# shionhonda/IaGo

Hardware: AMD Instinct MI355X
Metric: self-play games/sec (higher is better)
Workload: dtype f16 MFMA operands (float32 split in 2 / 3 pieces), f32 accumulate; u64 bitboards; f32 / f64 tree statistics

## Files before the change

iago_amd/csrc/search_kernel.hip:

```cpp
#include "mcts_dev.hpp"
#include "conv_trunk_body.hpp"
#include "conv_policy_body.hpp"
#include "sample_dev.hpp"
#include "search_request.hpp"
#include "../../include/iago_hip_serving.h"

#include <algorithm>
#include <cstdlib>
#include <mutex>
#include <string>
#include <vector>

namespace {
using namespace iago;
using namespace iago_mcts;

typedef unsigned long long u64;
#define RLX_AGENT __ATOMIC_RELAXED, __HIP_MEMORY_SCOPE_AGENT

constexpr uint32_t QCAP = IAGO_SEARCH_QUEUE_ENTRIES;
constexpr int CTL_FINISHED = 2, CTL_ABORT = 3;
__host__ __device__ constexpr int ctl_head(uint32_t q) { return 8 + 2 * (int)q; }
__host__ __device__ constexpr int ctl_tail(uint32_t q) { return 9 + 2 * (int)q; }
enum { ST_READY = 0, ST_WAIT_PRIOR, ST_PRIOR_READY, ST_ROLL, ST_ROLL_FRESH, ST_WAIT_VALUE, ST_HAVE_VALUE, ST_DONE, ST_TURN, ST_MOVE,
       ST_WAIT_DRAW, ST_DRAW,
       ST_IDLE };
constexpr int CTL_NO_CHILDREN = 4;
constexpr uint32_t MATCH_KEY = 0x4D415443u;
constexpr int CTL_BAD_DRAW = 13;
constexpr int CTL_PROGRESS = 5, CTL_PLAYING = 6;
constexpr int CTL_NET_WGS = 7;
constexpr int CTL_IDLE = 14;
constexpr int CTL_NEXT_GAME = 12;
namespace rq = iago_request;
using rq::KIND_POLICY;
using rq::KIND_VALUE;
using rq::NOBODY;
constexpr int GAMES_PER_WG = IAGO_SEARCH_GAMES_PER_WORKGROUP;

constexpr int SEARCH_IMG_V = iago_trunk::lds_alloc(2) + iago_trunk::head_lds(2);
constexpr int SEARCH_IMG_P = iago_policy::BS + 1024 + iago_policy::HEAD_FLOATS * 4;
constexpr int SEARCH_IMG_TOP = SEARCH_IMG_V > SEARCH_IMG_P ? SEARCH_IMG_V : SEARCH_IMG_P;

struct SearchParams {
    Tree T;
    const uint64_t *root_own, *root_opp;
    const uint8_t *active;
    float c_puct, lmbda;
    int32_t n_thr, n_sims, n_game_wgs, games_per_wg;
    int32_t *cur_node;
    uint64_t *cur_own, *cur_opp;
    int32_t *path;
    int32_t path_stride;
    int32_t *done;
    uint8_t *roll;
    int8_t *z;
    float *leaf_value;
    int8_t *z_log;
    int32_t *z_log_n;
    int32_t z_log_rows;
    u64 *q_slots;
    uint32_t *ctl;
    u64 *rep_v, *rep_p;
    int64_t *totals;
    int32_t *stats;
    uint64_t *wg_own, *wg_opp;
    long long clock_limit;
    int32_t max_turns;
    uint64_t *game_own, *game_opp;
    int32_t *n_turns;
    uint64_t *rec_own, *rec_opp;
    uint8_t *rec_valid;
    int8_t *rec_move;
    int32_t *rec_pi;
    int32_t games_total, stream;
    u64 *vtable;
    uint32_t vtable_mask;
    int64_t *trace;
    int32_t trace_rows;
    int32_t policy_xcds;
    int32_t pair_backlog;
    int32_t pace_margin, pace_backlog;
    int32_t ahead_idle;
    int32_t roll_defer;
    int32_t path_lds_cap;
    int32_t wave;
    float vloss;
    int64_t n_slots;
    int64_t *wave_timing;
    int32_t park_empties;
    uint8_t *parked;
    int32_t *park_stones;
    uint8_t *park_pass;
    int32_t explore_turns;
    int32_t cap_fast, cap_full_256;
    int32_t chain_skip;
    uint16_t *noise_counts;
    int32_t noise_eps, noise_lg;
    int32_t forced_k_256;
    int32_t negamax;
    float prior_off;
    double visit_off;
};

__device__ __forceinline__ u64 ld(const u64 *p) { return __hip_atomic_load(p, RLX_AGENT); }
__device__ __forceinline__ void st(u64 *p, u64 x) { __hip_atomic_store(p, x, RLX_AGENT); }

__device__ __forceinline__ u64 *ring_entry(const SearchParams &S, uint32_t q, uint32_t t)
{
    return S.q_slots + ((u64)q * QCAP + t % QCAP) * (u64)rq::SLOT_STRIDE;
}

__device__ __forceinline__ void send_request(const SearchParams &S, uint32_t kind, int64_t g, uint32_t reply_tag,
                                             uint64_t own, uint64_t opp)
{
    const uint32_t t = __hip_atomic_fetch_add(&S.ctl[ctl_tail(kind)], 1u, RLX_AGENT);
    u64 *e = S.q_slots + ((u64)kind * QCAP + t % QCAP) * (u64)rq::SLOT_STRIDE;
    st(e + rq::W_TAG, rq::entry_word(t, reply_tag));
    st(e + rq::W_OWN_LO, rq::entry_word(t, (uint32_t)own));
    st(e + rq::W_OWN_HI, rq::entry_word(t, (uint32_t)(own >> 32)));
    st(e + rq::W_OPP_LO, rq::entry_word(t, (uint32_t)opp));
    st(e + rq::W_OPP_HI, rq::entry_word(t, (uint32_t)(opp >> 32)));
    st(e + rq::W_WHO, rq::entry_word(t, rq::who_word(kind, (uint32_t)g)));
    atomicAdd((unsigned long long *)&S.totals[(uint32_t)g == NOBODY ? 11 : kind], 1ull);
}

__device__ __forceinline__ bool search_over(const SearchParams &S, const long long t0)
{
    bool out = false;
    if (threadIdx.x == 0)
        out = __hip_atomic_load(&S.ctl[CTL_FINISHED], RLX_AGENT) >= (uint32_t)S.n_game_wgs ||
              __hip_atomic_load(&S.ctl[CTL_ABORT], RLX_AGENT) != 0u || wall_clock64() - t0 > S.clock_limit;
    return __builtin_amdgcn_ballot_w64(out) != 0ull;
}

__device__ __forceinline__ int ring_backlog(const SearchParams &S, uint32_t q)
{
    int d = 0;
    if (threadIdx.x == 0)
        d = (int32_t)(__hip_atomic_load(&S.ctl[ctl_tail(q)], RLX_AGENT) - __hip_atomic_load(&S.ctl[ctl_head(q)], RLX_AGENT));
    return __builtin_amdgcn_readfirstlane(d);
}
__device__ __forceinline__ uint32_t ring_take(const SearchParams &S, uint32_t q)
{
    uint32_t t = 0;
    if (threadIdx.x == 0)
        t = __hip_atomic_fetch_add(&S.ctl[ctl_head(q)], 1u, RLX_AGENT);
    return __builtin_amdgcn_readfirstlane(t);
}
__device__ __forceinline__ int ring_fetch(const SearchParams &S, uint32_t q, uint32_t t, uint32_t max_spins, uint32_t *dst,
                                          const long long t0)
{
    const int tid = threadIdx.x;
    const u64 *e = ring_entry(S, q, t);
    u64 x = 0;
    int status = 0;
    for (uint32_t spins = 0;; spins++) {
        x = (tid < rq::WORDS) ? ld(e + tid) : 0ull;
        const bool ok = tid >= rq::WORDS || rq::entry_is(x, t);
        if (__builtin_amdgcn_ballot_w64(ok) == ~0ull)
            break;
        if (max_spins && spins + 1u >= max_spins) {
            status = 1;
            break;
        }
        if ((spins & 15u) == 15u && search_over(S, t0)) {
            status = 2;
            break;
        }
        __builtin_amdgcn_s_sleep(8);
    }
    if (status == 0 && tid < rq::WORDS)
        dst[tid] = (uint32_t)x;
    return status;
}

__device__ __forceinline__ void reply_value(const SearchParams &S, const uint32_t *r, uint32_t bits)
{
    if (rq::game(r) != NOBODY)
        st(&S.rep_v[(int64_t)rq::game(r)], rq::reply_word(rq::tag(r), bits));
}
__device__ __forceinline__ void reply_prior(const SearchParams &S, const uint32_t *r, int i, uint32_t bits)
{
    st(&S.rep_p[(int64_t)rq::game(r) * 64 + i], rq::reply_word(rq::tag(r), bits));
}

__device__ __forceinline__ uint32_t vtable_slot(const SearchParams &S, uint64_t own, uint64_t opp)
{
    uint64_t h = own * 0x9E3779B97F4A7C15ull ^ (opp + 0xD1B54A32D192ED03ull) * 0xBF58476D1CE4E5B9ull;
    h ^= h >> 29;
    h *= 0x94D049BB133111EBull;
    h ^= h >> 32;
    return (uint32_t)h & S.vtable_mask;
}

__device__ __forceinline__ bool vtable_get(const SearchParams &S, uint64_t own, uint64_t opp, uint32_t &bits, uint32_t &writer)
{
    const u64 *e = S.vtable + (u64)vtable_slot(S, own, opp) * 4u;
    const u64 s1 = ld(e), o = ld(e + 1), p = ld(e + 2), v = ld(e + 3);
    __builtin_amdgcn_fence(__ATOMIC_ACQUIRE, "wavefront");
    const u64 s2 = ld(e);
    bits = (uint32_t)v;
    writer = (uint32_t)(s1 >> 32);
    return s1 != 0ull && (s1 & 1ull) == 0ull && s1 == s2 && o == own && p == opp && (v >> 32) == (s1 & 0xFFFFFFFFull);
}

__device__ __forceinline__ u64 *vtable_put_begin(const SearchParams &S, uint64_t own, uint64_t opp, uint32_t bits, uint32_t writer,
                                                 u64 &publish)
{
    u64 *e = S.vtable + (u64)vtable_slot(S, own, opp) * 4u;
    const u64 s = __hip_atomic_fetch_or(e, 1ull, RLX_AGENT);
    if (s & 1ull)
        return nullptr;
    uint32_t seq = (uint32_t)s + 2u;
    seq = seq ? seq : 2u;
    st(e + 1, own);
    st(e + 2, opp);
    st(e + 3, ((u64)seq << 32) | bits);
    publish = ((u64)writer << 32) | seq;
    return e;
}
__device__ __forceinline__ void vtable_put_end(u64 *e, u64 publish)
{
    asm volatile("s_waitcnt vmcnt(0)" ::: "memory");
    st(e, publish);
}

template <int CTRL>
__device__ __forceinline__ void most_visited_step(int &n, int &a)
{
    const int on = (int)dpp_u32<CTRL>((uint32_t)n), oa = (int)dpp_u32<CTRL>((uint32_t)a);
    const bool take = on > n || (on == n && oa < a);
    n = take ? on : n;
    a = take ? oa : a;
}

__device__ __forceinline__ bool group8_all(bool x)
{
    return group8_add(x ? 0u : 1u) == 0u;
}

__device__ __forceinline__ int policy_draw(const u64 *rep, uint64_t lg, double u)
{
    double s = 0.0;
#pragma unroll 1
    for (int j = 0; j < 64; j++)
        s += ((lg >> j) & 1ull) ? (double)__uint_as_float(rq::reply_bits(ld(rep + j))) : 0.0;
    double last = 0.0;
#pragma unroll 1
    for (int j = 0; j < 64; j++)
        last += (((lg >> j) & 1ull) ? (double)__uint_as_float(rq::reply_bits(ld(rep + j))) : 0.0) / s;
    if (!(s > 0.0) || !(s <= 1.7976931348623157e308) || !(last > 0.0))
        return 64;
    double acc = 0.0;
    int n = 0;
#pragma unroll 1
    for (int j = 0; j < 64; j++) {
        acc += (((lg >> j) & 1ull) ? (double)__uint_as_float(rq::reply_bits(ld(rep + j))) : 0.0) / s;
        n += acc / last <= u ? 1 : 0;
    }
    return n;
}

__device__ __forceinline__ int path_entry(int path_at, const int32_t *gpath, int d)
{
    return path_at >= 0 ? ((const int32_t *)iago_trunk::trunk_lds)[path_at + d] : gpath[d];
}

template <bool WAVE>
__device__ __forceinline__ void backup_game(const SearchParams &S, int64_t g, uint32_t r, int leaf, bool fresh, float vg,
                                            int path_n, const int8_t zl, const int negamax, const int path_at,
                                            const int64_t gt)
{
    const int64_t base = gt * (int64_t)S.T.capacity;
    const float lmbda = S.lmbda;
    if (fresh && lmbda < 1.0f && r == 0u)
        S.T.nodes[base + leaf].v = vg;
    const int8_t zg = lmbda > 0.0f ? zl : (int8_t)0;
    const float lv = leaf_mix(lmbda, vg, zg);
    if (r == 0u) {
        S.leaf_value[g] = lv;
        if (S.z_log && lmbda > 0.0f)
            log_z(S.z_log, S.z_log_n, S.z_log_rows, gt, S.T.n_games, zg);
    }
    const int len = path_n < S.path_stride ? path_n : S.path_stride;
    const int32_t *const gpath = S.path + g * (int64_t)S.path_stride;
    const float lvd = backup_value(negamax, lv, path_n, (int)r);
    for (int d = (int)r; d < len; d += 8) {
        const int node = path_entry(path_at, gpath, d);
        visit(S.T, base + node, lvd);
        if constexpr (WAVE)
            S.T.nodes[base + node].reserved1 -= 1;
    }
}

__device__ __forceinline__ bool wg_handoff_or(bool x)
{
    __builtin_amdgcn_fence(__ATOMIC_RELEASE, "workgroup");
    const bool any = __syncthreads_or(x) != 0;
    __builtin_amdgcn_fence(__ATOMIC_ACQUIRE, "workgroup");
    return any;
}


struct Slot {
    int tid, gl;
    int wg;
    uint32_t r;
    Lane8 L;
    bool mine, exists;
    int64_t g, gt, base;
    int64_t n_slots;
    int W, s_in, tl;
    int path_at;
    int32_t *gpath;
    bool whole, need_v, need_z;
    int search_end;
};

struct Game {
    int state;
    uint32_t epoch;
    int n_done, turn, stones;
    bool pass_flg, g_over;
    uint64_t g_own, g_opp;
};

struct Cursor {
    int node, fc, k, nv, nvv;
    uint32_t vbits;
    uint64_t own, opp;
    int path_n, leaf;
    bool may_expand, leaf_fresh;
    float v_reply;
};

struct GameLds {
    uint64_t h_own[GAMES_PER_WG], h_opp[GAMES_PER_WG];
    int32_t h_stream[GAMES_PER_WG];
    int32_t h_game[GAMES_PER_WG];
    int32_t h_budget[GAMES_PER_WG];
    uint8_t h_fast[GAMES_PER_WG];
    uint32_t wg_count[7];
    int32_t ch_from[GAMES_PER_WG], ch_len[GAMES_PER_WG], ch_run[GAMES_PER_WG];
    int32_t roll_list[GAMES_PER_WG];
    uint32_t roll_wave[BLOCK / 64], roll_wave_old[BLOCK / 64];
    int32_t pace[4];
    uint32_t claimed;
    int32_t negamax;
    int8_t h_z[GAMES_PER_WG];
};
template <bool WAVE> struct GameShared : GameLds {};
template <> struct GameShared<true> : GameLds {
    int32_t wv_next[GAMES_PER_WG], wv_size[GAMES_PER_WG], wv_block[GAMES_PER_WG];
    long long wv_time[4];
};

template <bool WAVE>
__device__ __forceinline__ Slot make_slot(const SearchParams &S, const int wg)
{
    Slot I;
    I.wg = wg;
    I.tid = threadIdx.x;
    I.gl = I.tid >> 3;
    I.L = make_lane8(threadIdx.x);
    I.r = I.L.l8;
    I.mine = I.tid < 8 * S.games_per_wg;
    I.g = (int64_t)wg * S.games_per_wg + I.gl;
    I.W = WAVE ? S.wave : 1;
    I.n_slots = WAVE ? S.n_slots : S.T.n_games;
    I.exists = I.mine && I.g < I.n_slots;
    I.gt = WAVE ? I.g / I.W : I.g;
    I.s_in = WAVE ? (int)(I.g % I.W) : 0;
    I.tl = WAVE ? I.gl / I.W : 0;
    I.base = I.exists ? I.gt * (int64_t)S.T.capacity : 0;
    I.need_v = S.lmbda < 1.0f;
    I.need_z = S.lmbda > 0.0f;
    const bool path_lds = (size_t)S.games_per_wg * (size_t)S.path_stride * 4u <= (size_t)S.path_lds_cap;
    I.path_at = path_lds ? I.gl * S.path_stride : -1;
    I.gpath = S.path + (I.exists ? I.g : 0) * (int64_t)S.path_stride;
    I.whole = S.max_turns > 0;
    I.search_end = I.whole ? ST_MOVE : ST_DONE;
    return I;
}

__device__ __forceinline__ void start_game(Game &G, uint64_t own, uint64_t opp)
{
    G.g_own = own;
    G.g_opp = opp;
    G.turn = 0;
    G.stones = 4;
    G.pass_flg = false;
    G.g_over = false;
    G.n_done = 0;
}

template <bool WAVE>
__device__ __forceinline__ void cursor_to(Cursor &C, int node, uint32_t fc, uint32_t nv, uint32_t an, uint32_t vv, uint32_t vbits)
{
    C.node = node;
    C.fc = (int)fc;
    C.k = (int)((an >> 8) & 0xFFu);
    C.nv = (int)nv;
    if (WAVE)
        C.nvv = (int)vv;
    C.vbits = vbits;
}

__device__ __forceinline__ void finish_playout(const SearchParams &S, const Slot &I, const GameLds &sh, Game &G,
                                               const Cursor &C, bool fresh, float v)
{
    backup_game<false>(S, I.g, I.r, C.leaf, fresh, v, C.path_n, sh.h_z[I.gl], sh.negamax, I.path_at, I.g);
    G.n_done++;
    if (S.trace && I.r == 0u)
        atomicAdd((unsigned long long *)&S.totals[9], 1ull);
    if (I.r == 0u)
        S.done[I.g] = G.turn * S.n_sims + G.n_done;
    G.state = G.n_done >= sh.h_budget[I.gl] ? I.search_end : ST_READY;
}

__device__ __forceinline__ void take_replies(const SearchParams &S, const iago_row::HwParams &R, const Slot &I,
                                             const GameLds &sh, Game &G, Cursor &C)
{
    if (G.state == ST_WAIT_PRIOR || G.state == ST_WAIT_DRAW) {
        bool ok = true;
#pragma unroll
        for (int i = 0; i < 8; i++)
            ok = ok && rq::reply_tag(ld(&S.rep_p[I.g * 64 + (int)I.r * 8 + i])) == G.epoch;
        if (group8_all(ok)) {
            if (G.state == ST_WAIT_DRAW) {
                const uint64_t lg = group8_legal(to_lane(G.g_own, I.L), to_lane(G.g_opp, I.L), I.L);
                const double u = sample_uniform(R.key0, R.key1 ^ MATCH_KEY, R.id_base + (uint32_t)sh.h_game[I.gl],
                                                (uint32_t)G.turn, 0u);
                C.leaf = policy_draw(S.rep_p + I.g * 64, lg, u);
                if (C.leaf == 64) {
                    if (I.r == 0u)
                        __hip_atomic_store(&S.ctl[CTL_BAD_DRAW], 1u, RLX_AGENT);
                    C.leaf = (int)__builtin_ctzll(lg);
                }
            }
            G.state = G.state == ST_WAIT_PRIOR ? ST_PRIOR_READY : ST_DRAW;
        }
    } else if (G.state == ST_WAIT_VALUE) {
        const u64 x = ld(&S.rep_v[I.g]);
        if (rq::reply_tag(x) == G.epoch) {
            C.v_reply = __uint_as_float(rq::reply_bits(x));
            G.state = ST_HAVE_VALUE;
        }
    }
}

__device__ __forceinline__ int most_visited(const Tree &T, const Slot &I, uint64_t lg, int rfc, bool at_move, int (&row_n)[8])
{
    int best_n = -1, best_a = 0x7fffffff;
#pragma unroll
    for (int i = 0; i < 8; i++) {
        const int a = (int)(8u * I.r) + i;
        int n = 0;
        if (at_move && rfc >= 0 && ((lg >> a) & 1ull)) {
            n = T.nodes[I.base + rfc + __popcll(lg & ((1ull << a) - 1ull))].n_visits;
            if (n > best_n) {
                best_n = n;
                best_a = a;
            }
        }
        row_n[i] = n;
    }
    most_visited_step<DPP_XOR1>(best_n, best_a);
    most_visited_step<DPP_XOR2>(best_n, best_a);
    most_visited_step<DPP_HALF_MIRROR>(best_n, best_a);
    return best_n >= 0 ? best_a : -2;
}

__device__ __forceinline__ void record_turn(const SearchParams &S, const Slot &I, const GameLds &sh, const Game &G, int valid,
                                            int mv, const int (&row_n)[8])
{
    const int64_t row = (int64_t)G.turn * S.games_total + sh.h_game[I.gl];
    if (I.r == 0u) {
        S.rec_own[row] = G.g_own;
        S.rec_opp[row] = G.g_opp;
        S.rec_valid[row] = (uint8_t)valid;
        S.rec_move[row] = (int8_t)(valid ? mv : -1);
    }
#pragma unroll
    for (int i = 0; i < 8; i++)
        S.rec_pi[row * 64 + (int)(8u * I.r) + i] = row_n[i];
}

__device__ __forceinline__ void advance_root(const Tree &T, const Slot &I, uint64_t lg, int rfc, int mv)
{
    int child = -1;
    if (rfc >= 0) {
        if (mv >= 0 && ((lg >> mv) & 1ull))
            child = rfc + __popcll(lg & ((1ull << mv) - 1ull));
        else if (mv == -1 && (int)T.nodes[I.base + rfc].action == -1)
            child = rfc;
    }
    if (child >= 0) {
        T.root[I.g] = child;
        T.nodes[I.base + child].parent = -1;
    } else {
        fresh_root(T, I.g, I.base);
    }
}

__device__ __forceinline__ void play_move(const SearchParams &S, const Slot &I, const GameLds &sh, Game &G, bool played, int mv,
                                          const long long t0)
{
    place_stone(G.g_own, G.g_opp, mv, I.L);
    const bool was_over = G.g_over;
    G.stones += played ? 1 : 0;
    const bool passing = !played && !was_over;
    if (passing && G.pass_flg)
        G.stones = 64;
    if (!was_over)
        G.pass_flg = passing;
    if (G.turn % 2 == 1)
        G.g_over = was_over || G.stones >= 64;
    G.turn++;
    if (G.turn >= S.max_turns || (G.turn % 2 == 0 && G.g_over)) {
        if (I.r == 0u) {
            const int64_t id = sh.h_game[I.gl];
            S.n_turns[id] = G.turn;
// ... 402 lines not shown
    }
    const int n_roll = __popc(gm), rem = n_roll & 15;
    const int n_now = (n_roll < 16 || rem > S.roll_defer) ? n_roll : n_roll - rem;
    const uint32_t below = (1u << I.gl) - 1u;
    const int rank = deferred ? __popc(go & below) : __popc(go) + __popc(gm & ~go & below);
    const bool now = rolls && rank < n_now;
    if (now && I.r == 0u)
        sh.roll_list[rank] = (int32_t)I.g;
    deferred = rolls && !now;
    __syncthreads();
    if (I.tid == 0)
        sh.wg_count[2 + (n_roll == 0 ? 0 : n_roll <= 16 ? 1 : n_roll <= 20 ? 2 : 3)]++;
    const iago_row::RowHandoff hand = {sh.h_own, sh.h_opp, sh.h_stream, sh.h_game, sh.h_z,
                                       (int32_t)((int64_t)I.wg * S.games_per_wg)};
#pragma unroll 1
    for (int at = 0; at < n_now; at += 16) {
        iago_row::rollout_row_body<false, true, true>(R, 0u, sh.roll_list + at, table_ready, &hand);
        table_ready = true;
        __syncthreads();
    }
    return !rolls || now;
}

__device__ __forceinline__ void wave_backups(const SearchParams &S, const Slot &I, GameShared<true> &sh, Game &G,
                                             const Cursor &C, const long long c_roll, bool &busy)
{
    const long long c_back = wall_clock64();
    if (I.tid == 0)
        sh.wv_time[1] += c_back - c_roll;
    if (I.mine && I.r == 0u && G.state != ST_HAVE_VALUE && G.state != ST_DONE && I.s_in < sh.wv_size[I.tl])
        sh.wv_block[I.tl] = 1;
    __syncthreads();
    const bool ready = I.mine && G.state != ST_DONE && sh.wv_block[I.tl] == 0;
    if (wg_handoff_or(ready)) {
        for (int j = 0; j < I.W; j++) {
            if (ready && I.s_in == j && G.state == ST_HAVE_VALUE) {
                backup_game<true>(S, I.g, I.r, C.leaf, C.leaf_fresh, C.v_reply, C.path_n, sh.h_z[I.gl], sh.negamax, I.path_at, I.gt);
                if (S.trace && I.r == 0u)
                    atomicAdd((unsigned long long *)&S.totals[9], 1ull);
            }
            wg_handoff_or(false);
        }
        if (ready) {
            G.n_done += sh.wv_size[I.tl];
            const int m = S.n_sims - G.n_done < I.W ? S.n_sims - G.n_done : I.W;
            G.state = G.n_done >= S.n_sims ? ST_DONE : (I.s_in < m ? ST_READY : ST_IDLE);
            if (I.r == 0u)
                S.done[I.g] = G.n_done;
            busy = true;
        }
        __syncthreads();
        if (ready && I.s_in == 0 && I.r == 0u) {
            const int m = S.n_sims - G.n_done < I.W ? S.n_sims - G.n_done : I.W;
            sh.wv_size[I.tl] = m;
            sh.wv_next[I.tl] = 0;
        }
    }
    if (I.mine && I.r == 0u && I.s_in == 0)
        sh.wv_block[I.tl] = 0;
    if (I.tid == 0)
        sh.wv_time[2] += wall_clock64() - c_back;
}

__device__ __forceinline__ bool iteration_end(const SearchParams &S, const Slot &I, GameLds &sh, const Game &G,
                                              const CtlWords &c, const long long t0, int &contrib, bool &in_play)
{
    const Tree &T = S.T;
    if (S.trace && I.wg == 0 && I.tid == 0 && (int64_t)sh.wg_count[0] < S.trace_rows - T.n_games) {
        const int64_t iters = (int64_t)sh.wg_count[0];
        S.trace[4 * iters + 0] = wall_clock64() - t0;
        S.trace[4 * iters + 1] = __hip_atomic_load(&S.ctl[ctl_tail(0)], RLX_AGENT) + __hip_atomic_load(&S.ctl[ctl_tail(1)], RLX_AGENT);
        S.trace[4 * iters + 2] = __hip_atomic_load(&S.ctl[ctl_head(0)], RLX_AGENT) + __hip_atomic_load(&S.ctl[ctl_head(1)], RLX_AGENT);
        S.trace[4 * iters + 3] = (int64_t)__hip_atomic_load(&S.ctl[CTL_FINISHED], RLX_AGENT) |
                                 (__hip_atomic_load(&S.totals[9], RLX_AGENT) << 8);
    }
    if (I.tid == 0)
        sh.wg_count[0]++;
    const int prog = G.state == ST_DONE ? 0 : G.turn * S.n_sims + G.n_done;
    if (I.mine && I.r == 0u) {
        if (prog != contrib)
            atomicAdd(&sh.pace[0], prog - contrib);
        if (in_play && G.state == ST_DONE)
            atomicAdd(&sh.pace[1], -1);
    }
    contrib = prog;
    in_play = in_play && G.state != ST_DONE;
    const bool over = wall_clock64() - t0 > S.clock_limit;
    if (over && I.tid == 0)
        __hip_atomic_store(&S.ctl[CTL_ABORT], 1u, RLX_AGENT);
    const int stop = __syncthreads_or(over || (I.tid == 0 && c.abort != 0u));
    if (I.tid == 0) {
        if (sh.pace[0])
            __hip_atomic_fetch_add(&S.ctl[CTL_PROGRESS], (uint32_t)sh.pace[0], RLX_AGENT);
        if (sh.pace[1])
            __hip_atomic_fetch_add(&S.ctl[CTL_PLAYING], (uint32_t)sh.pace[1], RLX_AGENT);
        sh.pace[0] = 0;
        sh.pace[1] = 0;
        int limit = 0x7fffffff;
        sh.pace[3] = 0;
        const int32_t wait0 = (int32_t)(c.t0 - c.h0), wait1 = (int32_t)(c.t1 - c.h1);
        if (S.ahead_idle >= 0 && S.vtable && I.n_slots <= (int64_t)(QCAP / 2u) && c.idle >= (uint32_t)S.ahead_idle &&
            wait0 <= 0 && wait1 <= 0)
            sh.pace[3] = (int32_t)((QCAP - (uint32_t)I.n_slots) / 2u) / S.n_game_wgs;
        if (S.pace_margin >= 0 && (!S.stream || (int64_t)c.next + T.n_games >= (int64_t)S.games_total)) {
            if (wait0 + wait1 > S.pace_backlog && c.play != 0u && c.play <= (uint32_t)T.n_games)
                limit = (int)(c.prog / c.play) + S.pace_margin;
        }
        sh.pace[2] = limit;
    }
    return stop != 0;
}

__device__ __forceinline__ bool stream_claim(const SearchParams &S, const Slot &I, GameLds &sh, Game &G, bool &in_play)
{
    const Tree &T = S.T;
    const int n_here = (int)min((int64_t)S.games_per_wg, I.n_slots - (int64_t)I.wg * S.games_per_wg);
    if (I.tid == 0)
        sh.claimed = __hip_atomic_fetch_add(&S.ctl[CTL_NEXT_GAME], (uint32_t)n_here, RLX_AGENT);
    __syncthreads();
    const int64_t next = T.n_games + (int64_t)sh.claimed + I.gl;
    if (I.exists && next < S.games_total) {
        start_game(G, S.game_own[next], S.game_opp[next]);
        if (I.r == 0u) {
            S.done[I.g] = 0;
            fresh_root(T, I.g, I.base);
            atomicAdd(&sh.pace[1], 1);
        }
        sh.h_game[I.gl] = (int32_t)next;
        sh.ch_from[I.gl] = -1;
        G.state = ST_TURN;
        in_play = true;
    }
    return __syncthreads_and(!I.mine || G.state == ST_DONE) != 0;
}

template <bool WAVE>
__device__ __forceinline__ void epilogue(const SearchParams &S, const Slot &I, GameShared<WAVE> &sh, const Game &G,
                                         int st_levels, int st_children, const long long t0)
{
    if (I.exists && I.r == 0u && S.stats) {
        if (WAVE) {
            atomicAdd(&S.stats[2 * I.gt], st_levels);
            atomicAdd(&S.stats[2 * I.gt + 1], st_children);
        } else {
            S.stats[2 * I.g] += st_levels;
            S.stats[2 * I.g + 1] += st_children;
        }
    }
    if constexpr (WAVE) {
        if (I.tid < 4 && S.wave_timing)
            atomicAdd((unsigned long long *)&S.wave_timing[I.tid], (unsigned long long)sh.wv_time[I.tid]);
    }
    if (I.exists && I.r == 0u && G.state != ST_DONE && __hip_atomic_load(&S.ctl[CTL_ABORT], RLX_AGENT) != 0u) {
        S.cur_node[I.g] = (int32_t)G.epoch;
        S.leaf_value[I.g] = (float)G.state;
    }
    if (I.tid == 0) {
        atomicAdd((unsigned long long *)&S.totals[2], (unsigned long long)sh.wg_count[0]);
        atomicAdd((unsigned long long *)&S.totals[6], (unsigned long long)sh.wg_count[1]);
        atomicAdd((unsigned long long *)&S.totals[10], (unsigned long long)sh.wg_count[2]);
        atomicAdd((unsigned long long *)&S.totals[13], (unsigned long long)sh.wg_count[3]);
        atomicAdd((unsigned long long *)&S.totals[14], (unsigned long long)sh.wg_count[4]);
        atomicAdd((unsigned long long *)&S.totals[15], (unsigned long long)sh.wg_count[5]);
        if (S.chain_skip)
            atomicAdd((unsigned long long *)&S.totals[16], (unsigned long long)sh.wg_count[6]);
        atomicAdd((unsigned long long *)&S.totals[7], (unsigned long long)(wall_clock64() - t0));
        __hip_atomic_fetch_add(&S.ctl[CTL_FINISHED], 1u, RLX_AGENT);
    }
}

template <bool WAVE, bool PARK = false, bool NOISE = false>
__device__ __forceinline__ void game_workgroup(const SearchParams &S, const iago_row::HwParams &R, const long long t0, const int wg)
{
    __shared__ GameShared<WAVE> sh;
    const Slot I = make_slot<WAVE>(S, wg);
    const bool first = I.exists && I.gt < S.games_total && (S.stream || S.active[I.gt] != 0);
    Game G;
    G.state = (first && S.n_sims > 0) ? (I.whole ? ST_TURN : ST_READY) : ST_DONE;
    G.epoch = 0u;
    if constexpr (WAVE) {
        const int m = S.n_sims < I.W ? S.n_sims : I.W;
        if (G.state == ST_READY && I.s_in >= m)
            G.state = ST_IDLE;
        if (I.tid < GAMES_PER_WG) {
            sh.wv_next[I.tid] = 0;
            sh.wv_size[I.tid] = m;
            sh.wv_block[I.tid] = 0;
        }
        if (I.tid < 4)
            sh.wv_time[I.tid] = 0;
    }
    if (I.exists && I.r == 0u) {
        S.done[I.g] = 0;
        S.roll[I.g] = 0;
    }
    if (I.mine) {
        sh.h_game[I.gl] = (int32_t)I.gt;
        sh.h_budget[I.gl] = S.n_sims;
        sh.h_fast[I.gl] = 0;
        sh.ch_from[I.gl] = -1;
    }
    const bool whole_game = I.whole && I.exists && I.g < S.games_total;
    start_game(G, whole_game ? S.game_own[I.g] : 0ull, whole_game ? S.game_opp[I.g] : 0ull);
    if (whole_game && G.state == ST_DONE && I.r == 0u)
        S.n_turns[I.g] = 0;
    Cursor C = {};
    C.fc = -1;
    int st_levels = 0, st_children = 0;
    if (I.tid < 7)
        sh.wg_count[I.tid] = 0u;
    if (I.tid == 7)
        sh.negamax = S.negamax;
    bool deferred = false;
    bool table_ready = false;
    int contrib = 0;
    bool in_play = G.state != ST_DONE;
    if (I.tid < 4)
        sh.pace[I.tid] = I.tid == 2 ? 0x7fffffff : 0;
    __syncthreads();
    if (I.mine && in_play && I.r == 0u)
        atomicAdd(&sh.pace[1], 1);
    int pace_limit = 0x7fffffff;

    for (;;) {
        const long long c_it = WAVE ? wall_clock64() : 0;
        bool busy = false;
        if (I.mine) {
            take_replies(S, R, I, sh, G, C);
            if (!WAVE && G.state == ST_HAVE_VALUE) {
                finish_playout(S, I, sh, G, C, true, C.v_reply);
                busy = true;
            }
            if (!WAVE && I.whole)
                turn_boundary<PARK>(S, R, I, sh, G, C, busy, t0);
        }
        const long long c_desc = WAVE ? wall_clock64() : 0;
        for (int sub = 0; sub < (WAVE ? I.W : 1); sub++) {
            bool went = false;
            if (I.mine) {
                went = descend<WAVE, NOISE>(S, I, sh, G, C, pace_limit, st_levels, st_children);
                busy = busy || went;
            }
            if constexpr (WAVE) {
                if (!wg_handoff_or(went))
                    break;
            }
        }
        if constexpr (WAVE) {
            if (I.tid == 0)
                sh.wv_time[0] += wall_clock64() - c_desc;
        }
        const CtlWords c = read_ctl(S, I.tid);
        const bool rolls = I.mine && I.need_z && (G.state == ST_ROLL || G.state == ST_ROLL_FRESH);
        const long long c_roll = WAVE ? wall_clock64() : 0;
        const bool rolled = rollout_passes(S, R, I, sh, rolls, deferred, table_ready);
        if (I.mine && rolled) {
            if (G.state == ST_ROLL) {
                if constexpr (WAVE) {
                    C.v_reply = __uint_as_float(C.vbits);
                    G.state = ST_HAVE_VALUE;
                } else {
                    finish_playout(S, I, sh, G, C, C.leaf_fresh, __uint_as_float(C.vbits));
                }
            } else if (G.state == ST_ROLL_FRESH) {
                G.state = ST_WAIT_VALUE;
            }
        }
        if constexpr (WAVE)
            wave_backups(S, I, sh, G, C, c_roll, busy);
        const bool stop = iteration_end(S, I, sh, G, c, t0, contrib, in_play);
        bool all_done = __syncthreads_and(!I.mine || G.state == ST_DONE) != 0;
        pace_limit = sh.pace[2];
        if (all_done && !stop && S.stream)
            all_done = stream_claim(S, I, sh, G, in_play);
        if (all_done || stop)
            break;
        if (!__syncthreads_or(busy)) {
            if (I.tid == 0)
                sh.wg_count[1]++;
            __builtin_amdgcn_s_sleep(32);
            if constexpr (WAVE) {
                if (I.tid == 0)
                    sh.wv_time[3] += wall_clock64() - c_it;
            }
        }
    }
    epilogue<WAVE>(S, I, sh, G, st_levels, st_children, t0);
}


struct NetLds {
    uint32_t req[2][rq::WORDS];
    uint32_t status, count;
    float res_v[2], res_p[64];
};
struct NetWeights {
    float *w1_val, *w1_pol;
    char *head_v;
    float *head_p;
};
struct NetState {
    uint32_t carry;
    int n_carry;
    u64 *put_e;
    u64 put_word;
    long long t_wait, t_walk, n_pairs;
};

__device__ __forceinline__ NetWeights stage_net_weights(const iago_trunk::TrunkRParams &VP, const iago_policy::PolicyParams &PP)
{
    const int tid = threadIdx.x;
    float *const w1_val = (float *)(iago_trunk::trunk_lds + SEARCH_IMG_TOP), *const w1_pol = w1_val + (64 * 18 + 64);
    for (int e = tid; e < 64 * 18 / 4; e += 256) {
        ((float4 *)w1_val)[e] = ((const float4 *)VP.w1)[e];
        ((float4 *)w1_pol)[e] = ((const float4 *)PP.w1)[e];
    }
    if (tid < 16) {
        ((float4 *)(w1_val + 64 * 18))[tid] = ((const float4 *)VP.b1)[tid];
        ((float4 *)(w1_pol + 64 * 18))[tid] = ((const float4 *)PP.b1)[tid];
    }
    char *const head_v = (char *)(w1_pol + (64 * 18 + 64));
    float *const head_p = (float *)(head_v + iago_trunk::HEAD_W_LDS);
    for (int e = tid; e < 512; e += 256) {
        ((uint4 *)head_v)[e] = VP.w9_hi[e];
        ((uint4 *)(head_v + iago_trunk::HEAD_W_W9LO))[e] = VP.w9_lo[e];
    }
    for (int e = tid; e < 128 * 16; e += 256)
        ((float4 *)(head_v + iago_trunk::HEAD_W_W10))[(e & 15) * 128 + (e >> 4)] = ((const float4 *)VP.w10)[e];
    if (tid < 128)
        ((float *)(head_v + iago_trunk::HEAD_W_W11))[tid] = VP.w11[tid];
    if (tid == 0)
        *(float *)(head_v + iago_trunk::HEAD_W_B9) = VP.b9[0];
    if (tid < 128)
        head_p[tid] = PP.w9[tid];
    if (tid < 64)
        head_p[128 + tid] = PP.b10[tid];
    __syncthreads();
    return NetWeights{w1_val, w1_pol, head_v, head_p};
}

__device__ __forceinline__ void claim(const SearchParams &S, const uint32_t home, NetState &N, NetLds &L, const long long t0)
{
    const int tid = threadIdx.x;
    int status = 2, count = 0;
    bool polling = false;
    for (;;) {
        uint32_t q = home;
        bool have = N.n_carry > 0;
        uint32_t t1 = N.carry;
        if (have) {
            q = KIND_VALUE;
            N.n_carry = 0;
        } else if (ring_backlog(S, home) > 0) {
            t1 = ring_take(S, home);
            have = true;
        } else if (ring_backlog(S, home ^ 1u) > 0) {
            q = home ^ 1u;
            t1 = ring_take(S, q);
            have = true;
        }
        if (have) {
            status = ring_fetch(S, q, t1, 0u, L.req[0], t0);
            count = status == 0 ? 1 : 0;
            if (status == 0 && q == KIND_VALUE && ring_backlog(S, KIND_VALUE) >= S.pair_backlog) {
                const uint32_t t2 = ring_take(S, KIND_VALUE);
                if (ring_fetch(S, KIND_VALUE, t2, 8u, L.req[1], t0) == 0) {
                    count = 2;
                } else {
                    N.carry = t2;
                    N.n_carry = 1;
                }
            }
            break;
        }
        if (search_over(S, t0))
            break;
        if (!polling) {
            polling = true;
            if (tid == 0)
                __hip_atomic_fetch_add(&S.ctl[CTL_IDLE], 1u, RLX_AGENT);
        }
        __builtin_amdgcn_s_sleep(16);
    }
    if (polling && tid == 0)
        __hip_atomic_fetch_add(&S.ctl[CTL_IDLE], 0xFFFFFFFFu, RLX_AGENT);
    if (tid == 0) {
        L.status = (uint32_t)status;
        L.count = (uint32_t)count;
    }
}

__device__ __forceinline__ void answer_value(const SearchParams &S, const iago_trunk::TrunkRParams &VP, NetState &N, NetLds &L,
                                             const NetWeights &Wt, const int64_t row0, const int count)
{
    const int tid = threadIdx.x;
    iago_trunk::Piece W = iago_trunk::whole_walk(VP);
    W.pos = L.req[0];
    W.res = L.res_v;
    W.w1s = Wt.w1_val;
    W.head_w = Wt.head_v;
    if (count == 2)
        iago_trunk::trunk_item<true, 2, true>(VP, W, row0, row0 + count);
    else
        iago_trunk::trunk_item<true, 1, true>(VP, W, row0, row0 + count);
    __syncthreads();
    if (tid < count) {
        const uint32_t *r = L.req[tid];
        const uint32_t bits = __float_as_uint(L.res_v[tid]);
        reply_value(S, r, bits);
        if (S.vtable)
            N.put_e = vtable_put_begin(S, rq::own(r), rq::opp(r), bits, rq::game(r) != NOBODY ? rq::game(r) : rq::tag(r),
                                       N.put_word);
    }
}

__device__ __forceinline__ void answer_policy(const SearchParams &S, const iago_policy::PolicyParams &PP, NetLds &L,
                                              const NetWeights &Wt, const int64_t row0)
{
    const int tid = threadIdx.x;
    iago_policy::policy_item<true>(PP, row0, L.req[0], L.res_p, Wt.w1_pol, Wt.head_p);
    __syncthreads();
    if (tid < 64)
        reply_prior(S, L.req[0], tid, __float_as_uint(L.res_p[tid]));
}

__device__ __forceinline__ void leave(const SearchParams &S, const NetState &N)
{
    if (threadIdx.x == 0) {
        atomicAdd((unsigned long long *)&S.totals[3], (unsigned long long)N.n_pairs);
        atomicAdd((unsigned long long *)&S.totals[4], (unsigned long long)N.t_wait);
        atomicAdd((unsigned long long *)&S.totals[5], (unsigned long long)N.t_walk);
    }
}

__device__ __forceinline__ void net_workgroup(const SearchParams &S, const iago_trunk::TrunkRParams &VP,
                                              const iago_policy::PolicyParams &PP, const long long t0, const int wg)
{
    __shared__ __align__(16) NetLds L;
    const int tid = threadIdx.x;
    const int64_t row0 = 4 * (int64_t)wg;
    const uint32_t home = ((int)((uint32_t)wg & 7u) >= 8 - S.policy_xcds) ? KIND_POLICY : KIND_VALUE;
    NetState N = {0u, 0, nullptr, 0, 0, 0, 0};
    const NetWeights Wt = stage_net_weights(VP, PP);
    for (;;) {
        const long long c0 = wall_clock64();
        if (N.put_e) {
            vtable_put_end(N.put_e, N.put_word);
            N.put_e = nullptr;
        }
        if (tid < 64)
            claim(S, home, N, L, t0);
        __syncthreads();
        const long long c1 = wall_clock64();
        N.t_wait += c1 - c0;
        if (L.status != 0u) {
            leave(S, N);
            return;
        }
        const uint32_t kind = rq::kind(L.req[0]);
        const int count = (int)L.count;
        N.n_pairs += count - 1;
        if (kind == KIND_VALUE)
            answer_value(S, VP, N, L, Wt, row0, count);
        else
            answer_policy(S, PP, L, Wt, row0);
        __syncthreads();
        N.t_walk += wall_clock64() - c1;
    }
}

template <bool WAVE, bool PARK = false, bool NOISE = false>
__device__ __forceinline__ void search_body(const SearchParams &S, const iago_row::HwParams &R, const iago_trunk::TrunkRParams &VP,
                                            const iago_policy::PolicyParams &PP)
{
    const long long t0 = wall_clock64();
    const int wg = (int)blockIdx.x;
    if (wg == 0 && threadIdx.x == 0)
        __hip_atomic_store(&S.ctl[CTL_NET_WGS], (uint32_t)gridDim.x - (uint32_t)S.n_game_wgs, RLX_AGENT);
    if (wg < S.n_game_wgs)
        game_workgroup<WAVE, PARK, NOISE>(S, R, t0, wg);
    net_workgroup(S, VP, PP, t0, wg);
}

__global__ __launch_bounds__(256) __attribute__((amdgpu_waves_per_eu(1, 1))) void search_kernel(
    SearchParams S, iago_row::HwParams R, iago_trunk::TrunkRParams VP, iago_policy::PolicyParams PP)
{
    search_body<false>(S, R, VP, PP);
}

__global__ __launch_bounds__(256) __attribute__((amdgpu_waves_per_eu(1, 1))) void search_wave_kernel(
    SearchParams S, iago_row::HwParams R, iago_trunk::TrunkRParams VP, iago_policy::PolicyParams PP)
{
    search_body<true>(S, R, VP, PP);
}

__global__ __launch_bounds__(256) __attribute__((amdgpu_waves_per_eu(2, 2))) void search_game_kernel(SearchParams S,
                                                                                                   iago_row::HwParams R)
{
    game_workgroup<false>(S, R, wall_clock64(), (int)blockIdx.x);
}

__global__ __launch_bounds__(256) __attribute__((amdgpu_waves_per_eu(1, 1))) void search_park_kernel(
    SearchParams S, iago_row::HwParams R, iago_trunk::TrunkRParams VP, iago_policy::PolicyParams PP)
{
    search_body<false, true>(S, R, VP, PP);
}

__global__ __launch_bounds__(256) __attribute__((amdgpu_waves_per_eu(2, 2))) void search_game_park_kernel(SearchParams S,
                                                                                                        iago_row::HwParams R)
{
    game_workgroup<false, true>(S, R, wall_clock64(), (int)blockIdx.x);
}

__global__ __launch_bounds__(256) __attribute__((amdgpu_waves_per_eu(1, 1))) void search_noise_kernel(
    SearchParams S, iago_row::HwParams R, iago_trunk::TrunkRParams VP, iago_policy::PolicyParams PP)
{
    search_body<false, false, true>(S, R, VP, PP);
}

__global__ __launch_bounds__(256) __attribute__((amdgpu_waves_per_eu(2, 2))) void search_game_noise_kernel(SearchParams S,
                                                                                                         iago_row::HwParams R)
{
    game_workgroup<false, false, true>(S, R, wall_clock64(), (int)blockIdx.x);
}

__global__ __launch_bounds__(256) __attribute__((amdgpu_waves_per_eu(1, 1))) void search_net_kernel(
    SearchParams S, iago_trunk::TrunkRParams VP, iago_policy::PolicyParams PP)
{
    const long long t0 = wall_clock64();
    if (blockIdx.x == 0 && threadIdx.x == 0)
        __hip_atomic_store(&S.ctl[CTL_NET_WGS], (uint32_t)gridDim.x, RLX_AGENT);
    net_workgroup(S, VP, PP, t0, (int)blockIdx.x);
}

struct ArenaSet {
    SearchParams S;
    iago_row::HwParams R;
    iago_trunk::TrunkRParams VP;
    iago_policy::PolicyParams PP;
};
struct ArenaArgs {
    ArenaSet set[2];
};
static_assert(sizeof(ArenaArgs) <= 4096, "the arena's two parameter sets must fit the kernel argument segment");

__global__ __launch_bounds__(256) __attribute__((amdgpu_waves_per_eu(1, 1))) void search_arena_kernel(ArenaArgs P)
{
    const long long t0 = wall_clock64();
    const int b = (int)blockIdx.x;
    const int ga = P.set[0].S.n_game_wgs, games = ga + P.set[1].S.n_game_wgs;
    if (b == 0 && threadIdx.x == 0) {
        __hip_atomic_store(&P.set[0].S.ctl[CTL_NET_WGS], (uint32_t)gridDim.x - (uint32_t)games, RLX_AGENT);
        __hip_atomic_store(&P.set[1].S.ctl[CTL_NET_WGS], (uint32_t)gridDim.x - (uint32_t)games, RLX_AGENT);
    }
    const int home = b < games ? (b >= ga ? 1 : 0) : (b & 1);
    if (b < games) {
        const ArenaSet &X = P.set[home];
        game_workgroup<false>(X.S, X.R, t0, home ? b - ga : b);
    }
#pragma unroll 1
    for (int pass = 0; pass < 2; pass++) {
        const ArenaSet &X = P.set[home ^ pass];
        net_workgroup(X.S, X.VP, X.PP, t0, b);
    }
}

constexpr int search_lds() { return SEARCH_IMG_TOP + iago_trunk::W1_LDS + iago_policy::W1_LDS + iago_trunk::HEAD_W_LDS + 192 * 4; }

__global__ void search_scratch_warm_kernel(uint32_t *out, int n)
{
    volatile uint32_t a[64];
    for (int i = 0; i < 64; i++)
        a[i] = (uint32_t)(i * n) + threadIdx.x;
    uint32_t sum = 0;
    for (int i = 0; i < 64; i++)
        sum += a[(i * 7 + n) & 63];
    if (n == 0x7fffffff && out)
        out[0] = sum;
}

enum Form { F_SINGLE, F_WAVE, F_PARK, F_GAME, F_GAME_PARK, F_NET, F_ARENA, F_NOISE, F_GAME_NOISE, N_FORMS };

struct FormCache {
    const void *kernel;
    std::atomic<uint64_t> reserved{0};
    int static_lds = -1;
    struct {
        int lds = -1, per_cu = 0, cus = 0;
    } on[64];
} form_cache[N_FORMS] = {{(const void *)search_kernel},      {(const void *)search_wave_kernel},
                         {(const void *)search_park_kernel}, {(const void *)search_game_kernel},
                         {(const void *)search_game_park_kernel}, {(const void *)search_net_kernel},
                         {(const void *)search_arena_kernel},     {(const void *)search_noise_kernel},
                         {(const void *)search_game_noise_kernel}};
std::mutex form_cache_mutex;

int reserve_lds(Form f, int bytes, const char *who) { return iago_reserve_lds(form_cache[f].kernel, bytes, form_cache[f].reserved, who); }

bool static_lds_of(Form f, int &bytes)
{
    std::lock_guard<std::mutex> lock(form_cache_mutex);
    hipFuncAttributes fa;
    if (form_cache[f].static_lds < 0 && hipFuncGetAttributes(&fa, form_cache[f].kernel) == hipSuccess)
        form_cache[f].static_lds = (int)fa.sharedSizeBytes;
    bytes = form_cache[f].static_lds;
    return bytes >= 0;
}

bool residency_of(Form f, int dev, int lds, int &per_cu, int *cus)
{
    std::lock_guard<std::mutex> lock(form_cache_mutex);
    auto &r = form_cache[f].on[dev & 63];
    if (cus && r.cus < 1 && hipDeviceGetAttribute(&r.cus, hipDeviceAttributeMultiprocessorCount, dev) != hipSuccess) {
        r.cus = 0;
        return false;
    }
    if (r.lds != lds) {
        r.lds = -1;
        if (hipOccupancyMaxActiveBlocksPerMultiprocessor(&r.per_cu, form_cache[f].kernel, 256, (size_t)lds) != hipSuccess)
            return false;
        r.lds = lds;
    }
    per_cu = r.per_cu;
    if (cus)
        *cus = r.cus;
    return true;
}

}

extern "C" int iago_mcts_search_capacity(int32_t *cus, int32_t *workgroups_per_cu)
{
    if (!cus || !workgroups_per_cu)
        return iago_fail(IAGO_ERR_INVALID, "iago_mcts_search_capacity: null pointer");
    if (reserve_lds(F_SINGLE, search_lds(), "iago_mcts_search_capacity: cannot reserve the nets' LDS image"))
        return IAGO_ERR_HIP;
    int dev = 0, n_cu = 0, per = 0;
    if (hipGetDevice(&dev) != hipSuccess)
        return iago_fail(IAGO_ERR_HIP, "iago_mcts_search_capacity: hipGetDevice failed");
    if (!residency_of(F_SINGLE, dev, search_lds(), per, &n_cu))
        return iago_fail(IAGO_ERR_HIP, "iago_mcts_search_capacity: the device does not answer");
    if (n_cu < 1 || per < 1 || per > 255)
        return iago_fail(IAGO_ERR_CAPACITY, "iago_mcts_search_capacity: the search kernel does not fit a CU of this device");
    *cus = n_cu;
    *workgroups_per_cu = per;
    return IAGO_OK;
}

struct iago_search_streams {
    int device;
    int32_t cus, game_cus;
    hipStream_t game, net;
    hipEvent_t ready, game_done, net_done;
};

namespace {
struct LaunchRequest {
    iago_search_streams *streams = nullptr;
    const iago_search_wave_args *wave = nullptr;
    const iago_search_park_args *park = nullptr;
    int explore_turns = 0;
    int cap_fast = 0, cap_full_256 = 256;
    const iago_root_noise *noise = nullptr;
    int forced_k_256 = 0;
};

constexpr int SEARCH_FLAGS = IAGO_SEARCH_CHAIN_SKIP | IAGO_SEARCH_NEGAMAX | IAGO_SEARCH_PUCT_AZ;
int games_per_wg_of(const iago_mcts_search_args *a)
{
    return a->games_per_workgroup > 0 ? (a->games_per_workgroup & ~SEARCH_FLAGS) : a->games_per_workgroup;
}

int check_args(const iago_mcts_search_args *a, const iago_search_wave_args *wv)
{
    if (!a || !a->tree || !a->value || !a->policy || !a->rollout)
        return iago_fail(IAGO_ERR_INVALID, "iago_mcts_search_persistent: null args");
    const iago_mcts_tree *tree = a->tree;
    if (tree->n_games < 1 || tree->capacity < 1 || !tree->nodes || ((uintptr_t)tree->nodes & 31u) || !tree->n_nodes ||
        !tree->root || !tree->overflow || !tree->has_v)
        return iago_fail(IAGO_ERR_INVALID, "iago_mcts_search_persistent: bad tree (the value cache `v` is required)");
    if (tree->n_games > 0x7FFFFFF0ll)
        return iago_fail(IAGO_ERR_INVALID, "iago_mcts_search_persistent: too many games");
    if (!a->active || !a->cur_node || !a->cur_own || !a->cur_opp || !a->path ||
        a->path_stride < 8 || !a->done || !a->roll || !a->leaf_value || !a->q_slots || !a->ctl || !a->rep_v || !a->rep_p ||
        !a->totals || !a->wg_own || !a->wg_opp || ((uintptr_t)a->q_slots & 63u) || ((uintptr_t)a->rep_p & 7u) ||
        ((uintptr_t)a->rep_v & 7u) || ((uintptr_t)a->ctl & 15u))
        return iago_fail(IAGO_ERR_INVALID, "iago_mcts_search_persistent: null or misaligned state array");
    if (a->n_thr < 1 || a->n_sims < 0 || !(a->lmbda >= 0.0f && a->lmbda <= 1.0f) || a->net_workgroups < 1)
        return iago_fail(IAGO_ERR_INVALID, "iago_mcts_search_persistent: n_thr >= 1, n_sims >= 0, 0 <= lmbda <= 1, "
                                           "net_workgroups >= 1 expected");
    if (a->max_turns < 0 || (a->max_turns > 0 && (!a->game_own || !a->game_opp || !a->n_turns)) ||
        (a->max_turns > 0 && a->rec_move && (!a->rec_own || !a->rec_opp || !a->rec_valid || !a->rec_pi)))
        return iago_fail(IAGO_ERR_INVALID, "iago_mcts_search_persistent: whole games (max_turns > 0) need game_own, game_opp, "
                                           "n_turns, and all of rec_own / rec_opp / rec_valid / rec_move / rec_pi or none");
    if (a->games_total < 0 || (a->games_total > 0 && (a->max_turns == 0 || a->n_sims < 1 || a->z_log || a->z_log_rows > 0 ||
                                                      a->trace || a->trace_rows > 0)))
        return iago_fail(IAGO_ERR_INVALID, "iago_mcts_search_persistent: games_total >= 0; a stream (games_total > 0) plays "
                                           "whole games (max_turns > 0, n_sims >= 1), without z_log or trace");
    if (a->max_turns == 0 && (!a->root_own || !a->root_opp))
        return iago_fail(IAGO_ERR_INVALID, "iago_mcts_search_persistent: root_own / root_opp expected");
    if (a->z_log_rows > 0 && (!a->z_log || !a->z_log_n))
        return iago_fail(IAGO_ERR_INVALID, "iago_mcts_search_persistent: z_log needs z_log_n");
    const iago_rollout_args *ro = a->rollout;
    const int64_t n_slots = tree->n_games * (wv ? wv->width : 1);
    if (wv && n_slots > (int64_t)QCAP)
        return iago_fail(IAGO_ERR_CAPACITY, "iago_mcts_search_wave: more slots (n_games x width) than a request ring holds");
    if (ro->n != n_slots || !ro->z || !ro->table || ((uintptr_t)ro->table & 15u) || ro->log_form || ro->trace ||
        ro->uniforms || ro->throughput_hint != 0)
        return iago_fail(IAGO_ERR_INVALID, "iago_mcts_search_persistent: product-form rollout of the n games without "
                                           "trace / uniforms expected");
    const int gpw = games_per_wg_of(a);
    if (!wv && gpw > 0 && gpw != 8 && gpw != 16 && gpw != 24 && gpw != 32)
        return iago_fail(IAGO_ERR_INVALID, "iago_mcts_search_persistent: games_per_workgroup is 0 (= 32), 8, 16 or 32");
    if (a->max_cus < 0)
        return iago_fail(IAGO_ERR_INVALID, "iago_mcts_search_persistent: max_cus < 0");
    if (a->vtable_slots > 0 && (!a->vtable || ((uintptr_t)a->vtable & 31u) || (a->vtable_slots & (a->vtable_slots - 1)) != 0))
        return iago_fail(IAGO_ERR_INVALID, "iago_mcts_search_persistent: vtable must be 32-byte aligned, vtable_slots a "
                                           "power of two");
    return IAGO_OK;
}

struct SearchGrid {
    int gpw;
    int chain_skip;
    int negamax;
    int puct_az;
    int64_t n_slots, n_game_wgs, net_wgs, grid;
    int path_lds_cap, game_lds;
};

void size_games(const iago_mcts_search_args *a, const iago_search_wave_args *wv, SearchGrid &G)
{
    G.gpw = wv || games_per_wg_of(a) <= 0 ? GAMES_PER_WG : games_per_wg_of(a);
    G.chain_skip = (!wv && a->games_per_workgroup > 0 && (a->games_per_workgroup & IAGO_SEARCH_CHAIN_SKIP)) ? 1 : 0;
    G.negamax = (a->games_per_workgroup > 0 && (a->games_per_workgroup & IAGO_SEARCH_NEGAMAX)) ? 1 : 0;
    G.puct_az = (a->games_per_workgroup > 0 && (a->games_per_workgroup & IAGO_SEARCH_PUCT_AZ)) ? 1 : 0;
    G.n_slots = a->tree->n_games * (wv ? wv->width : 1);
    G.n_game_wgs = (G.n_slots + G.gpw - 1) / G.gpw;
    G.path_lds_cap = SEARCH_IMG_TOP;
    G.game_lds = 0;
}

int cus_to_count_on(int max_cus, int cus) { return max_cus > 0 && max_cus < cus ? max_cus : cus; }

int check_net_rows(const iago_mcts_search_args *a, int64_t grid, const char *msg)
{
    if (a->value->n < 4 * grid || a->policy->n < 4 * grid || a->value->planes || a->value->index || a->value->n_dev ||
        a->policy->index || a->policy->n_dev || !a->value->own || a->value->own != a->wg_own ||
        a->value->opp != a->wg_opp || a->policy->own != a->wg_own || a->policy->opp != a->wg_opp)
        return iago_fail(IAGO_ERR_INVALID, msg);
    return IAGO_OK;
}

int size_grid(const iago_mcts_search_args *a, const LaunchRequest &q, SearchGrid &G)
{
// ... 560 lines not shown
```

iago_amd/csrc/search_request.hpp:

```cpp
#pragma once
#include <stdint.h>

#include <hip/hip_runtime.h>

namespace iago_request {

enum Word {
    W_WHO = 0,
    W_TAG,
    W_OWN_LO, W_OWN_HI,
    W_OPP_LO, W_OPP_HI,
    WORDS
};
constexpr int SLOT_STRIDE = 8;
constexpr uint32_t NOBODY = 0x7FFFFFFFu;
constexpr uint32_t KIND_VALUE = 0u, KIND_POLICY = 1u;

__host__ __device__ __forceinline__ uint32_t who_word(uint32_t kind, uint32_t game) { return (kind << 31) | game; }
__host__ __device__ __forceinline__ uint32_t kind(const uint32_t *r) { return r[W_WHO] >> 31; }
__host__ __device__ __forceinline__ uint32_t game(const uint32_t *r) { return r[W_WHO] & 0x7FFFFFFFu; }
__host__ __device__ __forceinline__ uint32_t tag(const uint32_t *r) { return r[W_TAG]; }
__host__ __device__ __forceinline__ uint64_t own(const uint32_t *r) { return ((uint64_t)r[W_OWN_HI] << 32) | r[W_OWN_LO]; }
__host__ __device__ __forceinline__ uint64_t opp(const uint32_t *r) { return ((uint64_t)r[W_OPP_HI] << 32) | r[W_OPP_LO]; }

__host__ __device__ __forceinline__ unsigned long long entry_word(uint32_t t, uint32_t x)
{
    return ((unsigned long long)(t + 1u) << 32) | x;
}
__host__ __device__ __forceinline__ bool entry_is(unsigned long long x, uint32_t t) { return (uint32_t)(x >> 32) == t + 1u; }

__host__ __device__ __forceinline__ unsigned long long reply_word(uint32_t tag, uint32_t bits)
{
    return ((unsigned long long)tag << 32) | bits;
}
__host__ __device__ __forceinline__ uint32_t reply_tag(unsigned long long x) { return (uint32_t)(x >> 32); }
__host__ __device__ __forceinline__ uint32_t reply_bits(unsigned long long x) { return (uint32_t)x; }

}
```

Before: 2993.

## Batch ring control reads and overlap vtable put with claim atomics

The claim loop now reads all four ring head/tail counters in one batch of loads instead of several serial backlog queries, and decides which ring to take from and whether to pair a second value request from that one snapshot. The value-table insert, previously done right after answering, is deferred into the next claim so its atomic fetch-or and stores are issued alongside the ring atomics. The publish store runs on the first fetch miss, when going idle, or after the claim. This aims to hide global atomic latency on the network workgroups' critical path. The risk is decisions made on slightly stale counters and later publication of cached values.

```diff
diff --git a/iago_amd/csrc/search_kernel.hip b/iago_amd/csrc/search_kernel.hip
--- a/iago_amd/csrc/search_kernel.hip
+++ b/iago_amd/csrc/search_kernel.hip
@@ -134,22 +134,35 @@
     return __builtin_amdgcn_ballot_w64(out) != 0ull;
 }
 
-__device__ __forceinline__ int ring_backlog(const SearchParams &S, uint32_t q)
-{
-    int d = 0;
+__device__ __forceinline__ void ring_look_issue(const SearchParams &S, uint32_t (&c)[4])
+{
+    static_assert(ctl_head(0) == 8 && ctl_tail(0) == 9 && ctl_head(1) == 10 && ctl_tail(1) == 11, "ctl[8..11]: the rings");
+    if (threadIdx.x == 0) {
+#pragma unroll
+        for (int i = 0; i < 4; i++)
+            c[i] = __hip_atomic_load(&S.ctl[8 + i], RLX_AGENT);
+    }
+}
+__device__ __forceinline__ rq::Look ring_look(const uint32_t (&c)[4])
+{
+    rq::Look k;
+    k.head[0] = __builtin_amdgcn_readfirstlane(c[0]);
+    k.tail[0] = __builtin_amdgcn_readfirstlane(c[1]);
+    k.head[1] = __builtin_amdgcn_readfirstlane(c[2]);
+    k.tail[1] = __builtin_amdgcn_readfirstlane(c[3]);
+    return k;
+}
+__device__ __forceinline__ uint32_t ring_take_issue(const SearchParams &S, uint32_t q)
+{
+    uint32_t t = 0, lane_off = 0;
+    asm volatile("" : "+v"(lane_off));
     if (threadIdx.x == 0)
-        d = (int32_t)(__hip_atomic_load(&S.ctl[ctl_tail(q)], RLX_AGENT) - __hip_atomic_load(&S.ctl[ctl_head(q)], RLX_AGENT));
-    return __builtin_amdgcn_readfirstlane(d);
-}
-__device__ __forceinline__ uint32_t ring_take(const SearchParams &S, uint32_t q)
-{
-    uint32_t t = 0;
-    if (threadIdx.x == 0)
-        t = __hip_atomic_fetch_add(&S.ctl[ctl_head(q)], 1u, RLX_AGENT);
-    return __builtin_amdgcn_readfirstlane(t);
-}
+        t = __hip_atomic_fetch_add(&S.ctl[ctl_head(q) + lane_off], 1u, RLX_AGENT);
+    return t;
+}
+template <class F>
 __device__ __forceinline__ int ring_fetch(const SearchParams &S, uint32_t q, uint32_t t, uint32_t max_spins, uint32_t *dst,
-                                          const long long t0)
+                                          const long long t0, F &&first_miss)
 {
     const int tid = threadIdx.x;
     const u64 *e = ring_entry(S, q, t);
@@ -168,6 +181,8 @@
             status = 2;
             break;
         }
+        if (spins == 0u)
+            first_miss();
         __builtin_amdgcn_s_sleep(8);
     }
     if (status == 0 && tid < rq::WORDS)
@@ -205,20 +220,19 @@
     return s1 != 0ull && (s1 & 1ull) == 0ull && s1 == s2 && o == own && p == opp && (v >> 32) == (s1 & 0xFFFFFFFFull);
 }
 
-__device__ __forceinline__ u64 *vtable_put_begin(const SearchParams &S, uint64_t own, uint64_t opp, uint32_t bits, uint32_t writer,
+__device__ __forceinline__ u64 vtable_put_begin(u64 *e) { return __hip_atomic_fetch_or(e, 1ull, RLX_AGENT); }
+__device__ __forceinline__ bool vtable_put_store(u64 *e, u64 s, uint64_t own, uint64_t opp, uint32_t bits, uint32_t writer,
                                                  u64 &publish)
 {
-    u64 *e = S.vtable + (u64)vtable_slot(S, own, opp) * 4u;
-    const u64 s = __hip_atomic_fetch_or(e, 1ull, RLX_AGENT);
     if (s & 1ull)
-        return nullptr;
+        return false;
     uint32_t seq = (uint32_t)s + 2u;
     seq = seq ? seq : 2u;
     st(e + 1, own);
     st(e + 2, opp);
     st(e + 3, ((u64)seq << 32) | bits);
     publish = ((u64)writer << 32) | seq;
-    return e;
+    return true;
 }
 __device__ __forceinline__ void vtable_put_end(u64 *e, u64 publish)
 {
@@ -1227,6 +1241,7 @@
 struct NetState {
     uint32_t carry;
     int n_carry;
+    int n_put;
     u64 *put_e;
     u64 put_word;
     long long t_wait, t_walk, n_pairs;
@@ -1264,32 +1279,62 @@
     return NetWeights{w1_val, w1_pol, head_v, head_p};
 }
 
+__device__ __forceinline__ void publish_put(NetState &N)
+{
+    if (N.put_e) {
+        vtable_put_end(N.put_e, N.put_word);
+        N.put_e = nullptr;
+    }
+}
+
 __device__ __forceinline__ void claim(const SearchParams &S, const uint32_t home, NetState &N, NetLds &L, const long long t0)
 {
     const int tid = threadIdx.x;
     int status = 2, count = 0;
     bool polling = false;
+    u64 *put = nullptr;
+    uint64_t put_own = 0, put_opp = 0;
+    uint32_t put_bits = 0, put_writer = 0;
+    if (tid < N.n_put) {
+        const uint32_t *r = L.req[tid];
+        put_own = rq::own(r);
+        put_opp = rq::opp(r);
+        put_bits = __float_as_uint(L.res_v[tid]);
+        put_writer = rq::game(r) != NOBODY ? rq::game(r) : rq::tag(r);
+        put = S.vtable + (u64)vtable_slot(S, put_own, put_opp) * 4u;
+    }
+    N.n_put = 0;
     for (;;) {
-        uint32_t q = home;
-        bool have = N.n_carry > 0;
-        uint32_t t1 = N.carry;
-        if (have) {
-            q = KIND_VALUE;
+        uint32_t c[4] = {0u, 0u, 0u, 0u};
+        ring_look_issue(S, c);
+        u64 seq_word = 1ull;
+        if (put)
+            seq_word = vtable_put_begin(put);
+        const rq::Look look = ring_look(c);
+        const bool carried = N.n_carry > 0;
+        const int take = rq::claim_plan(look, home, carried);
+        const uint32_t q = carried ? KIND_VALUE : (uint32_t)take;
+        uint32_t ticket = 0;
+        if (take != rq::TAKE_NONE)
+            ticket = ring_take_issue(S, q);
+        if (put) {
+            if (vtable_put_store(put, seq_word, put_own, put_opp, put_bits, put_writer, N.put_word))
+                N.put_e = put;
+            put = nullptr;
+        }
+        const uint32_t took = __builtin_amdgcn_readfirstlane(ticket);
+        if (carried || take != rq::TAKE_NONE) {
+            const uint32_t t1 = carried ? N.carry : took;
             N.n_carry = 0;
-        } else if (ring_backlog(S, home) > 0) {
-            t1 = ring_take(S, home);
-            have = true;
-        } else if (ring_backlog(S, home ^ 1u) > 0) {
-            q = home ^ 1u;
-            t1 = ring_take(S, q);
-            have = true;
-        }
-        if (have) {
-            status = ring_fetch(S, q, t1, 0u, L.req[0], t0);
+            const bool second = rq::claim_second(look, q, t1, S.pair_backlog);
+            uint32_t ticket2 = 0;
+            if (second)
+                ticket2 = ring_take_issue(S, KIND_VALUE);
+            status = ring_fetch(S, q, t1, 0u, L.req[0], t0, [&] { publish_put(N); });
             count = status == 0 ? 1 : 0;
-            if (status == 0 && q == KIND_VALUE && ring_backlog(S, KIND_VALUE) >= S.pair_backlog) {
-                const uint32_t t2 = ring_take(S, KIND_VALUE);
-                if (ring_fetch(S, KIND_VALUE, t2, 8u, L.req[1], t0) == 0) {
+            if (second) {
+                const uint32_t t2 = __builtin_amdgcn_readfirstlane(ticket2);
+                if (status == 0 && ring_fetch(S, KIND_VALUE, t2, 8u, L.req[1], t0, [] {}) == 0) {
                     count = 2;
                 } else {
                     N.carry = t2;
@@ -1302,6 +1347,7 @@
             break;
         if (!polling) {
             polling = true;
+            publish_put(N);
             if (tid == 0)
                 __hip_atomic_fetch_add(&S.ctl[CTL_IDLE], 1u, RLX_AGENT);
         }
@@ -1333,10 +1379,8 @@
         const uint32_t *r = L.req[tid];
         const uint32_t bits = __float_as_uint(L.res_v[tid]);
         reply_value(S, r, bits);
-        if (S.vtable)
-            N.put_e = vtable_put_begin(S, rq::own(r), rq::opp(r), bits, rq::game(r) != NOBODY ? rq::game(r) : rq::tag(r),
-                                       N.put_word);
-    }
+    }
+    N.n_put = S.vtable ? count : 0;
 }
 
 __device__ __forceinline__ void answer_policy(const SearchParams &S, const iago_policy::PolicyParams &PP, NetLds &L,
@@ -1365,17 +1409,14 @@
     const int tid = threadIdx.x;
     const int64_t row0 = 4 * (int64_t)wg;
     const uint32_t home = ((int)((uint32_t)wg & 7u) >= 8 - S.policy_xcds) ? KIND_POLICY : KIND_VALUE;
-    NetState N = {0u, 0, nullptr, 0, 0, 0, 0};
+    NetState N = {0u, 0, 0, nullptr, 0, 0, 0, 0};
     const NetWeights Wt = stage_net_weights(VP, PP);
     for (;;) {
         const long long c0 = wall_clock64();
-        if (N.put_e) {
-            vtable_put_end(N.put_e, N.put_word);
-            N.put_e = nullptr;
-        }
         if (tid < 64)
             claim(S, home, N, L, t0);
         __syncthreads();
+        publish_put(N);
         const long long c1 = wall_clock64();
         N.t_wait += c1 - c0;
         if (L.status != 0u) {
diff --git a/iago_amd/csrc/search_request.hpp b/iago_amd/csrc/search_request.hpp
--- a/iago_amd/csrc/search_request.hpp
+++ b/iago_amd/csrc/search_request.hpp
@@ -29,6 +29,36 @@
 }
 __host__ __device__ __forceinline__ bool entry_is(unsigned long long x, uint32_t t) { return (uint32_t)(x >> 32) == t + 1u; }
 
+struct Look {
+    uint32_t head[2], tail[2];
+};
+constexpr int TAKE_NONE = -1;
+
+__host__ __device__ __forceinline__ int32_t backlog(const Look &k, uint32_t q)
+{
+    return q ? (int32_t)(k.tail[1] - k.head[1]) : (int32_t)(k.tail[0] - k.head[0]);
+}
+
+__host__ __device__ __forceinline__ int claim_plan(const Look &k, uint32_t home, bool carried)
+{
+    if (carried)
+        return TAKE_NONE;
+    if (backlog(k, home) > 0)
+        return (int)home;
+    if (backlog(k, home ^ 1u) > 0)
+        return (int)(home ^ 1u);
+    return TAKE_NONE;
+}
+
+__host__ __device__ __forceinline__ bool claim_second(const Look &k, uint32_t q, uint32_t t1, int32_t pair_backlog)
+{
+    if (q != KIND_VALUE || (int32_t)(k.tail[KIND_VALUE] - t1) <= 0)
+        return false;
+    const uint32_t next = t1 + 1u;
+    const uint32_t from = (int32_t)(k.head[KIND_VALUE] - next) > 0 ? k.head[KIND_VALUE] : next;
+    return (int32_t)(k.tail[KIND_VALUE] - from) >= pair_backlog;
+}
+
 __host__ __device__ __forceinline__ unsigned long long reply_word(uint32_t tag, uint32_t bits)
 {
     return ((unsigned long long)tag << 32) | bits;
```

Result: no change. 2992 (-0.0%).
